# underdoc-wang/ST-MGCN

Hardware: AMD Instinct MI355X
Metric: train_samples_per_sec (higher is better)
Workload: dtype bf16; 1 GPU; model=ST_MGCN, preset=bench-1024, n_nodes=1024, seq_len=8, m_graphs=3, lstm_hidden=64, gcn_hidden=64, global_batch=32, parallelism=dp1, hipgraph=True, impl=hip

## Files before the change

### stmgcn_amd/csrc/wgrad.hip

```cpp

#include "common.h"

namespace {

template <int RB>
__device__ __forceinline__ int tswz(int g, int off) {
  return g * RB + (off ^ ((((unsigned)g / (256 / RB)) & (RB / 16 - 1)) << 4));
}

template <typename T, int RB>
__device__ __forceinline__ typename Frag8<T>::type frag_from(
    const char* lds_tile, int g, int koff_bytes) {
  return *(const typename Frag8<T>::type*)&lds_tile[tswz<RB>(g, koff_bytes)];
}

}

template <typename T>
struct LstmFin {
  unsigned* tickets;
  T* out;
  int gru, cin;
};

__host__ __device__ inline long lstm_grads_layer_off(int l, int GH, int cin) {
  return l == 0 ? 0 : (long)GH * (cin + 64 + 2) + (long)(l - 1) * GH * (64 + 64 + 2);
}

template <typename T, bool FIN>
__global__ void __launch_bounds__(512, 1)
lstm_wgrad_kernel(const T* __restrict__ dA, const T* __restrict__ hseq,
                  const T* __restrict__ x, float* __restrict__ dwih,
                  float* __restrict__ dwhh, float* __restrict__ db,
                  long R, long S_pad, int S, int Tst, int L, int cin1,
                  long tpc, LstmFin<T> fin) {
  using frag = typename Frag8<T>::type;
  constexpr int NTHR = 512;
  constexpr int MTG = 2;
  constexpr int KT = 64;
  constexpr int HT = 64 * 2 * KT;
  extern __shared__ char lds[];

  const int layer = blockIdx.y;
  const int wv = threadIdx.x >> 6, lane = threadIdx.x & 63;
  const int l16 = lane & 15, lgrp = lane >> 4;
  const int gw = wv * 32;
  const long ntile = R / SEQ_TILE;
  const long tb0 = (long)blockIdx.x * tpc;
  const long tb1 = (tb0 + tpc < ntile) ? tb0 + tpc : ntile;
  const long tp0 = S_pad / SEQ_TILE;
  if (!FIN && tb0 >= tb1) return;

  const T* dA_l = dA + (long)layer * R * STM_DA_GATES;
  const T* hp_l = hseq + (long)layer * R * 64;
  const T* hx_l = (layer > 0) ? hseq + (long)(layer - 1) * R * 64 : nullptr;
  const bool l0 = layer == 0;
  const bool x1 = cin1 && l0;

  f32x4 acc_hh[MTG][4], acc_ih[MTG][4];
  float dbp[MTG];
  #pragma unroll
  for (int mt = 0; mt < MTG; ++mt) {
    #pragma unroll
    for (int nt = 0; nt < 4; ++nt) acc_hh[mt][nt] = f32x4{0.f, 0.f, 0.f, 0.f};
    #pragma unroll
    for (int nt = 0; nt < 4; ++nt) acc_ih[mt][nt] = f32x4{0.f, 0.f, 0.f, 0.f};
    dbp[mt] = 0.f;
  }

  const int scb = threadIdx.x & 7, sp = (threadIdx.x >> 3) & 31;
  const int skh = sp >> 4, srow = stm_da_rho(2 * (sp & 15));
  const int sop = threadIdx.x >> 8;

  auto load_h = [&](long tb, frag v[2]) {
    const frag fz = {};
    const long tile = tb + skh;
    const long r = tile * SEQ_TILE + srow;
    v[0] = fz; v[1] = fz;
    if (tile >= tb1) return;
    if (sop == 0) {
      if (tile >= tp0) {
        v[0] = *(const frag*)&hp_l[(r - S_pad) * 64 + scb * 8];
        v[1] = *(const frag*)&hp_l[(r + 1 - S_pad) * 64 + scb * 8];
      }
    } else if (!l0) {
      v[0] = *(const frag*)&hx_l[r * 64 + scb * 8];
      v[1] = *(const frag*)&hx_l[(r + 1) * 64 + scb * 8];
    } else {
      const long s_ = r % S_pad, t_ = r / S_pad;
      if (x1) {
        if (scb == 0) {
          if (s_ < S) ((T*)&v[0])[0] = x[s_ * Tst + t_];
          if (s_ + 1 < S) ((T*)&v[1])[0] = x[(s_ + 1) * Tst + t_];
        }
      } else {
        if (s_ < S) v[0] = *(const frag*)&x[(s_ * Tst + t_) * 64 + scb * 8];
        if (s_ + 1 < S)
          v[1] = *(const frag*)&x[((s_ + 1) * Tst + t_) * 64 + scb * 8];
      }
    }
  };
  auto commit_h = [&](char* buf, const frag v[2]) {
    char* tileT = buf + sop * HT;
    #pragma unroll
    for (int j = 0; j < 8; ++j) {
      union { T t2[2]; int i; } pk;
      pk.t2[0] = ((const T*)&v[0])[j];
      pk.t2[1] = ((const T*)&v[1])[j];
      *(int*)&tileT[tswz<2 * KT>(scb * 8 + j, sp * 4)] = pk.i;
    }
  };
  auto load_a = [&](long tb, frag a[2][MTG]) {
    const frag fz = {};
    #pragma unroll
    for (int kh = 0; kh < 2; ++kh)
      #pragma unroll
      for (int mt = 0; mt < MTG; ++mt) {
        a[kh][mt] = fz;
        if (tb + kh < tb1)
          a[kh][mt] = *(const frag*)&dA_l[stm_da_tile_off((tb + kh) * SEQ_TILE) +
                                          stm_da_elem(gw + mt * 16 + l16, 8 * lgrp)];
      }
  };

  auto kstep = [&](long tb, char* buf, frag vs[2], frag a[2][MTG]) {
    char* hpT = buf;
    char* hxT = buf + HT;
    commit_h(buf, vs);
    load_h(tb + 4, vs);
    __syncthreads();
    #pragma unroll
    for (int kh = 0; kh < 2; ++kh) {
      const int koff = kh * KT + lgrp * 16;
      frag bh[4], bx[4];
      #pragma unroll
      for (int nt = 0; nt < 4; ++nt) bh[nt] = frag_from<T, 2 * KT>(hpT, nt * 16 + l16, koff);
      #pragma unroll
      for (int nt = 0; nt < 4; ++nt) bx[nt] = frag_from<T, 2 * KT>(hxT, nt * 16 + l16, koff);
      #pragma unroll
      for (int mt = 0; mt < MTG; ++mt) {
        const frag af = a[kh][mt];
        #pragma unroll
        for (int nt = 0; nt < 4; ++nt)
          acc_hh[mt][nt] = mfma16x16x32(af, bh[nt], acc_hh[mt][nt]);
        #pragma unroll
        for (int nt = 0; nt < 4; ++nt)
          acc_ih[mt][nt] = mfma16x16x32(af, bx[nt], acc_ih[mt][nt]);
        float sa = 0.f;
        #pragma unroll
        for (int j = 0; j < 8; ++j) sa += (float)af[j];
        dbp[mt] += sa;
      }
    }
    load_a(tb + 4, a);
  };

  frag vs0[2], vs1[2], a0[2][MTG], a1[2][MTG];
  load_h(tb0, vs0);
  load_a(tb0, a0);
  load_h(tb0 + 2, vs1);
  load_a(tb0 + 2, a1);
  for (long tb = tb0; tb < tb1; tb += 4) {
    kstep(tb, lds, vs0, a0);
    if (tb + 2 < tb1) kstep(tb + 2, lds + 2 * HT, vs1, a1);
  }


  float* whh = dwhh + (long)layer * 256 * 64;
  float* wih = dwih + (long)layer * 256 * 64;
  #pragma unroll
  for (int mt = 0; mt < MTG; ++mt) {
    #pragma unroll
    for (int nt = 0; nt < 4; ++nt)
      #pragma unroll
      for (int rr = 0; rr < 4; ++rr) {
        const int m = gw + mt * 16 + lgrp * 4 + rr;
        const int n = nt * 16 + l16;
        unsafeAtomicAdd(&whh[m * 64 + n], acc_hh[mt][nt][rr]);
        if (!x1 || n == 0)
          unsafeAtomicAdd(&wih[m * 64 + n], acc_ih[mt][nt][rr]);
      }
    float v = dbp[mt];
    v += __shfl_xor(v, 16, 64);
    v += __shfl_xor(v, 32, 64);
    if (lgrp == 0) unsafeAtomicAdd(&db[layer * 256 + gw + mt * 16 + l16], v);
  }

  if constexpr (FIN) {
    if (!stm_last_arriver(&fin.tickets[layer], gridDim.x, (int*)lds)) return;
    const int GH = fin.gru ? 192 : 256;
    const int cin_l = l0 ? fin.cin : 64;
    auto row_ih = [&](int m) { return m < GH ? m : -1; };
    auto row_hh = [&](int m) {
      return !fin.gru ? m : (m < 128 ? m : (m >= 192 ? m - 64 : -1));
    };
    T* o_ih = fin.out + lstm_grads_layer_off(layer, GH, fin.cin);
    T* o_hh = o_ih + (long)GH * cin_l;
    T* o_bi = o_hh + (long)GH * 64;
    T* o_bh = o_bi + GH;
    const float* dbl = db + layer * 256;
    constexpr int IT = 256 * 16 / NTHR;
    const bool dense = cin_l == 64;
    const int mb = threadIdx.x;
    float4 vh[IT], vi[IT];
    #pragma unroll
    for (int k = 0; k < IT; ++k) {
      const int i = threadIdx.x + k * NTHR;
      vh[k] = *(const float4*)&whh[i * 4];
      vi[k] = dense ? *(const float4*)&wih[i * 4] : float4{0.f, 0.f, 0.f, 0.f};
    }
    const float vb = mb < 256 ? dbl[mb] : 0.f;
    const float vc = (!dense && mb < 256) ? wih[mb * 64] : 0.f;
    #pragma unroll
    for (int k = 0; k < IT; ++k) {
      const int i = threadIdx.x + k * NTHR;
      const int m = i >> 4, n4 = (i & 15) * 4;
      const int rh = row_hh(m), ri = row_ih(m);
      if (rh >= 0)
        stm_store4<T>(&o_hh[rh * 64 + n4], vh[k].x, vh[k].y, vh[k].z, vh[k].w);
      if (dense && ri >= 0)
        stm_store4<T>(&o_ih[ri * 64 + n4], vi[k].x, vi[k].y, vi[k].z, vi[k].w);
    }
    if (mb >= 256) return;
    const int ri = row_ih(mb), rh = row_hh(mb);
    if (ri >= 0) o_bi[ri] = fromF<T>(vb);
    if (rh >= 0) o_bh[rh] = fromF<T>(vb);
    if (!dense && ri >= 0) o_ih[ri] = fromF<T>(vc);
  }
}

static void lstm_wgrad_launch(void* stream, int dtype, const void* dA,
                              const void* hseq, const void* x, float* dwih,
                              float* dwhh, float* db, long R, long S_pad,
                              int S, int Tst, int L, int cin,
                              unsigned* tickets, void* out, int gru) {
  static long env_chunks = -1;
  if (env_chunks < 0) {
    const char* e = getenv("STMGCN_WGRAD_CHUNKS");
    env_chunks = e ? atol(e) : 0;
  }
  if (R <= 0 || R % SEQ_TILE != 0) {
    printf("stmgcn_lstm_wgrad: R=%ld is not a whole number of dA tiles\n", R);
    return;
  }
  const long ntile = R / SEQ_TILE;
  const long target = env_chunks > 0 ? env_chunks : 512 / (L > 0 ? L : 1);
  long nchunks = (R + 1023) / 1024;
  if (nchunks > target) nchunks = target;
  if (nchunks < 1) nchunks = 1;
  const long tpc = (ntile + nchunks - 1) / nchunks;
  nchunks = (ntile + tpc - 1) / tpc;
  const size_t lds = 2 * 2 * 8192;
  stm_dispatch_lowp("stmgcn_lstm_wgrad", dtype, [&](auto t) {
    using T = decltype(t);
    const LstmFin<T> fin{tickets, (T*)out, gru, cin};
    stm_dispatch_bool(out != nullptr, [&](auto finc) {
      hipLaunchKernelGGL((lstm_wgrad_kernel<T, decltype(finc)::value>),
                         dim3((unsigned)nchunks, L), dim3(512), lds,
                         (hipStream_t)stream, (const T*)dA, (const T*)hseq,
                         (const T*)x, dwih, dwhh, db, R, S_pad, S, Tst, L,
                         cin == 1 ? 1 : 0, tpc, fin);
    });
  });
}

extern "C" void stmgcn_lstm_wgrad(void* stream, int dtype, const void* dA,
                                  const void* hseq, const void* x, float* dwih,
                                  float* dwhh, float* db, long R, long S_pad,
                                  int S, int Tst, int L, int cin) {
  lstm_wgrad_launch(stream, dtype, dA, hseq, x, dwih, dwhh, db, R, S_pad, S,
                    Tst, L, cin, nullptr, nullptr, 0);
}

extern "C" void stmgcn_lstm_wgrad_grads(void* stream, int dtype, const void* dA,
                                        const void* hseq, const void* x,
                                        float* dwih, float* dwhh, float* db,
                                        unsigned* tickets, void* out, long R,
                                        long S_pad, int S, int Tst, int L,
                                        int cin, int gru) {
  lstm_wgrad_launch(stream, dtype, dA, hseq, x, dwih, dwhh, db, R, S_pad, S,
                    Tst, L, cin, tickets, out, gru);
}

struct AtbSrc { const void* a[4]; };

template <typename T>
struct AtbFin {
  unsigned* ticket;
  T *dW, *dbo;
};

template <typename T, bool FIN>
__global__ void __launch_bounds__(256, 1)
atb_wgrad_kernel(AtbSrc As, int CA, const T* __restrict__ B,
                 float* __restrict__ C, float* __restrict__ db,
                 long rows, int M, int N, AtbFin<T> fin) {
  using frag = typename Frag8<T>::type;
  constexpr int KT = 64;
  constexpr int AT_B = 256 * 2 * KT;
  constexpr int BT_B = 64 * 2 * KT;
  constexpr int BUF_B = AT_B + BT_B;
  constexpr int NUA = 4;
  extern __shared__ char lds[];
  float* red = (float*)lds;
  const int wv = threadIdx.x >> 6, lane = threadIdx.x & 63;
  const int l16 = lane & 15, lgrp = lane >> 4;
  const long chunk = (rows + gridDim.x - 1) / gridDim.x;
  const long r0 = (long)blockIdx.x * chunk;
  const long r1 = (r0 + chunk < rows) ? r0 + chunk : rows;
  const int mtiles = (M + 15) / 16;
  const int ntiles = (N + 15) / 16;
  const int mt_mine = (mtiles - wv + 3) / 4;

  f32x4 acc[4][4];
  #pragma unroll
  for (int i = 0; i < 4; ++i)
    #pragma unroll
    for (int nt = 0; nt < 4; ++nt) acc[i][nt] = f32x4{0.f, 0.f, 0.f, 0.f};
  float dbp[8];
  #pragma unroll
  for (int j = 0; j < 8; ++j) dbp[j] = 0.f;

  const int ncba = mtiles * 2, ncbb = ntiles * 2;
  const T* ap[NUA];
  int apair[NUA], acb[NUA];
  #pragma unroll
  for (int i = 0; i < NUA; ++i) {
    const int u = threadIdx.x + i * 256;
    apair[i] = u / ncba; acb[i] = u % ncba;
    ap[i] = nullptr;
    if (u < 32 * ncba && acb[i] * 8 < M)
      ap[i] = (const T*)As.a[(acb[i] * 8) / CA] + (acb[i] * 8) % CA;
  }
  const int bpair = threadIdx.x / ncbb, bcb = threadIdx.x % ncbb;
  const bool bunit = threadIdx.x < 32 * ncbb;
  const T* bp = (bunit && bcb * 8 < N) ? B + bcb * 8 : nullptr;

  struct Regs { frag a[NUA][2]; frag b[2]; };
  auto load_tiles = [&](long kt, Regs& g) {
    const frag fz = {};
    #pragma unroll
    for (int i = 0; i < NUA; ++i) {
      g.a[i][0] = fz; g.a[i][1] = fz;
      const long ra = kt + apair[i] * 2;
      if (ap[i] != nullptr) {
        if (ra < r1) g.a[i][0] = *(const frag*)&ap[i][ra * CA];
        if (ra + 1 < r1) g.a[i][1] = *(const frag*)&ap[i][(ra + 1) * CA];
      }
    }
    g.b[0] = fz; g.b[1] = fz;
    const long rb = kt + bpair * 2;
    if (bp != nullptr) {
      if (rb < r1) g.b[0] = *(const frag*)&bp[rb * N];
      if (rb + 1 < r1) g.b[1] = *(const frag*)&bp[(rb + 1) * N];
    }
  };
  auto commit_tiles = [&](char* buf, const Regs& g) {
    char* AT = buf;
    char* BT = buf + AT_B;
    #pragma unroll
    for (int i = 0; i < NUA; ++i) {
      if (threadIdx.x + i * 256 < 32 * ncba) {
        #pragma unroll
        for (int j = 0; j < 8; ++j) {
          union { T t2[2]; int i; } pk;
          pk.t2[0] = ((const T*)&g.a[i][0])[j];
          pk.t2[1] = ((const T*)&g.a[i][1])[j];
          *(int*)&AT[tswz<2 * KT>(acb[i] * 8 + j, apair[i] * 4)] = pk.i;
        }
      }
    }
    if (bunit) {
      #pragma unroll
      for (int j = 0; j < 8; ++j) {
        union { T t2[2]; int i; } pk;
        pk.t2[0] = ((const T*)&g.b[0])[j];
        pk.t2[1] = ((const T*)&g.b[1])[j];
        *(int*)&BT[tswz<2 * KT>(bcb * 8 + j, bpair * 4)] = pk.i;
        if (db) dbp[j] += toF<T>(pk.t2[0]) + toF<T>(pk.t2[1]);
      }
    }
  };

  auto kstep = [&](long kt, char* buf, Regs& g) {
    commit_tiles(buf, g);
    load_tiles(kt + 2 * KT, g);
    __syncthreads();
    const char* AT = buf;
    const char* BT = buf + AT_B;
    #pragma unroll
    for (int kh = 0; kh < 2; ++kh) {
      const int koff = kh * KT + lgrp * 16;
      frag bf[4];
      #pragma unroll
      for (int nt = 0; nt < 4; ++nt)
        if (nt < ntiles) bf[nt] = frag_from<T, 2 * KT>(BT, nt * 16 + l16, koff);
      #pragma unroll
      for (int i = 0; i < 4; ++i) {
        if (i < mt_mine) {
          const frag a = frag_from<T, 2 * KT>(AT, (wv + i * 4) * 16 + l16, koff);
          #pragma unroll
          for (int nt = 0; nt < 4; ++nt)
            if (nt < ntiles) acc[i][nt] = mfma16x16x32(a, bf[nt], acc[i][nt]);
        }
      }
    }
  };

  Regs g0, g1;
  load_tiles(r0, g0);
  load_tiles(r0 + KT, g1);
  for (long kt = r0; kt < r1; kt += 2 * KT) {
    kstep(kt, lds, g0);
    if (kt + KT < r1) kstep(kt + KT, lds + BUF_B, g1);
  }
  __syncthreads();

  #pragma unroll
  for (int i = 0; i < 4; ++i) {
    if (i >= mt_mine) continue;
    const int mt = wv + i * 4;
    #pragma unroll
    for (int nt = 0; nt < 4; ++nt) {
      if (nt >= ntiles) continue;
      #pragma unroll
      for (int rr = 0; rr < 4; ++rr) {
        const int m = mt * 16 + lgrp * 4 + rr, n = nt * 16 + l16;
        if (m < M && n < N) unsafeAtomicAdd(&C[(long)m * N + n], acc[i][nt][rr]);
      }
    }
  }

  if (db) {
    #pragma unroll
    for (int j = 0; j < 8; ++j) red[threadIdx.x * 8 + j] = bunit ? dbp[j] : 0.f;
    __syncthreads();
    if (threadIdx.x < N) {
      const int n = threadIdx.x, cb = n >> 3, j = n & 7;
      float v = 0.f;
      for (int k = 0; k < 32; ++k) v += red[(k * ncbb + cb) * 8 + j];
      unsafeAtomicAdd(&db[n], v);
    }
  }

  if constexpr (FIN) {
    if (!stm_last_arriver(fin.ticket, gridDim.x, (int*)lds)) return;
    const int n4s = M * N / 4;
    for (int i0 = threadIdx.x; i0 < n4s; i0 += 4 * 256) {
      float4 v[4];
      #pragma unroll
      for (int k = 0; k < 4; ++k) {
        const int i = i0 + k * 256;
        v[k] = i < n4s ? *(const float4*)&C[i * 4] : float4{0.f, 0.f, 0.f, 0.f};
      }
      #pragma unroll
      for (int k = 0; k < 4; ++k) {
        const int i = i0 + k * 256;
        if (i < n4s) stm_store4<T>(&fin.dW[i * 4], v[k].x, v[k].y, v[k].z, v[k].w);
      }
    }
    if (db && threadIdx.x < N) fin.dbo[threadIdx.x] = fromF<T>(db[threadIdx.x]);
  }
}

static void atb_wgrad_launch(void* stream, int dtype, const void** As,
                             int nsrc, int CA, const void* B, float* C,
                             float* db, long rows, int N, unsigned* fin_ticket,
                             void* fin_dW, void* fin_db) {
  long nchunks = (rows + 255) / 256;
  if (nchunks > 512) nchunks = 512;
  if (nchunks < 1) nchunks = 1;
  const dim3 grid((unsigned)nchunks), blk(256);
  const size_t lds = 2 * (256 + 64) * 128;
  const int M = nsrc * CA;
  AtbSrc src{};
  for (int i = 0; i < nsrc && i < 4; ++i) src.a[i] = As[i];
  stm_dispatch_lowp("stmgcn_atb_wgrad", dtype, [&](auto t) {
    using T = decltype(t);
    const AtbFin<T> fin{fin_ticket, (T*)fin_dW, (T*)fin_db};
    stm_dispatch_bool(fin_ticket != nullptr, [&](auto finc) {
      STM_CHECK_HIP(hipFuncSetAttribute(
          (const void*)atb_wgrad_kernel<T, decltype(finc)::value>,
          hipFuncAttributeMaxDynamicSharedMemorySize, (int)lds));
      hipLaunchKernelGGL((atb_wgrad_kernel<T, decltype(finc)::value>), grid, blk,
                         lds, (hipStream_t)stream, src, CA, (const T*)B, C, db,
                         rows, M, N, fin);
    });
  });
}

extern "C" void stmgcn_atb_wgrad_multi(void* stream, int dtype, const void** As,
                                       int nsrc, int CA, const void* B, float* C,
                                       float* db, long rows, int N) {
  atb_wgrad_launch(stream, dtype, As, nsrc, CA, B, C, db, rows, N, nullptr,
                   nullptr, nullptr);
}

extern "C" void stmgcn_atb_wgrad_multi_grads(void* stream, int dtype,
                                             const void** As, int nsrc, int CA,
                                             const void* B, float* C, float* db,
                                             unsigned* ticket, void* dW,
                                             void* dbo, long rows, int N) {
  atb_wgrad_launch(stream, dtype, As, nsrc, CA, B, C, db, rows, N, ticket, dW,
                   dbo);
}

extern "C" void stmgcn_atb_wgrad(void* stream_v, int dtype, const void* A,
                                 const void* B, float* C, float* db, long rows,
                                 int M, int N) {
  stmgcn_atb_wgrad_multi(stream_v, dtype, &A, 1, M, B, C, db, rows, N);
}
```

Baseline: 16990 samples/s.

## Specialize LSTM wgrad loads per layer form and interleave LDS reads with MFMA

Splits the LSTM weight-gradient kernel into compile-time forms (scalar layer-0 input, dense layer-0 input, hidden handoff) so the h/x staging loads are branchless, with predicated addresses and masking applied at commit time. Adds sched_barrier fences so LDS fragment reads for the next k-half overlap with MFMAs on the current one. It also halves the default chunk target and drops the env override. The aim is to cut divergent branching and load-latency stalls in the inner loop, at the cost of extra registers and fewer blocks for atomics-based reduction parallelism.

```diff
diff --git a/stmgcn_amd/csrc/wgrad.hip b/stmgcn_amd/csrc/wgrad.hip
--- a/stmgcn_amd/csrc/wgrad.hip
+++ b/stmgcn_amd/csrc/wgrad.hip
@@ -12,6 +12,14 @@
 __device__ __forceinline__ typename Frag8<T>::type frag_from(
     const char* lds_tile, int g, int koff_bytes) {
   return *(const typename Frag8<T>::type*)&lds_tile[tswz<RB>(g, koff_bytes)];
+}
+
+enum : int { WG_SCALAR0 = 0, WG_DENSE0 = 1, WG_HANDOFF = 2 };
+template <typename F>
+__device__ __forceinline__ void wgrad_uniform_form(int form, F&& f) {
+  if (form == WG_SCALAR0) f(std::integral_constant<int, WG_SCALAR0>{});
+  else if (form == WG_DENSE0) f(std::integral_constant<int, WG_DENSE0>{});
+  else f(std::integral_constant<int, WG_HANDOFF>{});
 }
 
 }
@@ -70,101 +78,138 @@
 
   const int scb = threadIdx.x & 7, sp = (threadIdx.x >> 3) & 31;
   const int skh = sp >> 4, srow = stm_da_rho(2 * (sp & 15));
-  const int sop = threadIdx.x >> 8;
-
-  auto load_h = [&](long tb, frag v[2]) {
+  const bool sop = threadIdx.x >= 256;
+
+  struct KSet {
+    frag h[2];
+    unsigned short xs[2];
+    frag a[2][MTG];
+    int live;
+  };
+
+  auto load_h = [&](auto form, long tb, KSet& g) {
+    constexpr int F = decltype(form)::value;
+    const long tile = tb + skh;
+    const bool tin = tile < tb1;
+    const long r = tile * SEQ_TILE + srow;
+    const bool hlive = tin && tile >= tp0 && !(F == WG_SCALAR0 && sop);
+    const T* ph = hlive ? hp_l + (r - S_pad) * 64 : hp_l;
+    const T *p0 = ph, *p1 = ph + 64;
+    bool lv0 = hlive, lv1 = hlive;
+    if constexpr (F == WG_HANDOFF) {
+      const T* px = tin ? hx_l + r * 64 : hx_l;
+      p0 = sop ? px : p0; p1 = sop ? px + 64 : p1;
+      lv0 = lv1 = sop ? tin : hlive;
+    } else {
+      const long t_ = (unsigned)tile / (unsigned)tp0;
+      const long s_ = r - t_ * S_pad;
+      const bool x0 = sop && tin && s_ < S, x1 = sop && tin && s_ + 1 < S;
+      const long e0 = x0 ? s_ * Tst + t_ : 0, e1 = x1 ? (s_ + 1) * Tst + t_ : 0;
+      if constexpr (F == WG_DENSE0) {
+        p0 = sop ? x + e0 * 64 : p0; p1 = sop ? x + e1 * 64 : p1;
+      } else {
+        g.xs[0] = *(const unsigned short*)&x[e0];
+        g.xs[1] = *(const unsigned short*)&x[e1];
+      }
+      lv0 = sop ? x0 : hlive; lv1 = sop ? x1 : hlive;
+    }
+    g.h[0] = *(const frag*)&p0[scb * 8];
+    g.h[1] = *(const frag*)&p1[scb * 8];
+    g.live = (lv0 ? 1 : 0) | (lv1 ? 2 : 0);
+  };
+  auto commit_h = [&](auto form, char* buf, const KSet& g) {
+    constexpr int F = decltype(form)::value;
     const frag fz = {};
-    const long tile = tb + skh;
-    const long r = tile * SEQ_TILE + srow;
-    v[0] = fz; v[1] = fz;
-    if (tile >= tb1) return;
-    if (sop == 0) {
-      if (tile >= tp0) {
-        v[0] = *(const frag*)&hp_l[(r - S_pad) * 64 + scb * 8];
-        v[1] = *(const frag*)&hp_l[(r + 1 - S_pad) * 64 + scb * 8];
-      }
-    } else if (!l0) {
-      v[0] = *(const frag*)&hx_l[r * 64 + scb * 8];
-      v[1] = *(const frag*)&hx_l[(r + 1) * 64 + scb * 8];
-    } else {
-      const long s_ = r % S_pad, t_ = r / S_pad;
-      if (x1) {
-        if (scb == 0) {
-          if (s_ < S) ((T*)&v[0])[0] = x[s_ * Tst + t_];
-          if (s_ + 1 < S) ((T*)&v[1])[0] = x[(s_ + 1) * Tst + t_];
-        }
-      } else {
-        if (s_ < S) v[0] = *(const frag*)&x[(s_ * Tst + t_) * 64 + scb * 8];
-        if (s_ + 1 < S)
-          v[1] = *(const frag*)&x[((s_ + 1) * Tst + t_) * 64 + scb * 8];
-      }
-    }
-  };
-  auto commit_h = [&](char* buf, const frag v[2]) {
-    char* tileT = buf + sop * HT;
+    char* tileT = buf + (sop ? HT : 0);
+    const frag v0 = (g.live & 1) ? g.h[0] : fz;
+    const frag v1 = (g.live & 2) ? g.h[1] : fz;
+    const int xw = ((g.live & 1) ? (int)g.xs[0] : 0) |
+                   ((g.live & 2) ? (int)g.xs[1] << 16 : 0);
     #pragma unroll
     for (int j = 0; j < 8; ++j) {
-      union { T t2[2]; int i; } pk;
-      pk.t2[0] = ((const T*)&v[0])[j];
-      pk.t2[1] = ((const T*)&v[1])[j];
-      *(int*)&tileT[tswz<2 * KT>(scb * 8 + j, sp * 4)] = pk.i;
-    }
-  };
-  auto load_a = [&](long tb, frag a[2][MTG]) {
-    const frag fz = {};
+      union { typename Frag8<T>::elem t2[2]; int i; } pk;
+      pk.t2[0] = v0[j];
+      pk.t2[1] = v1[j];
+      int w = pk.i;
+      if constexpr (F == WG_SCALAR0) w = sop ? ((j == 0 && scb == 0) ? xw : 0) : w;
+      *(int*)&tileT[tswz<2 * KT>(scb * 8 + j, sp * 4)] = w;
+    }
+  };
+  auto load_a = [&](long tb, KSet& g) {
     #pragma unroll
     for (int kh = 0; kh < 2; ++kh)
       #pragma unroll
       for (int mt = 0; mt < MTG; ++mt) {
-        a[kh][mt] = fz;
-        if (tb + kh < tb1)
-          a[kh][mt] = *(const frag*)&dA_l[stm_da_tile_off((tb + kh) * SEQ_TILE) +
-                                          stm_da_elem(gw + mt * 16 + l16, 8 * lgrp)];
-      }
-  };
-
-  auto kstep = [&](long tb, char* buf, frag vs[2], frag a[2][MTG]) {
+        const long off = stm_da_tile_off((tb + kh) * SEQ_TILE) +
+                         stm_da_elem(gw + mt * 16 + l16, 8 * lgrp);
+        g.a[kh][mt] = *(const frag*)&dA_l[tb + kh < tb1 ? off : 0];
+      }
+  };
+
+  auto kstep = [&](auto form, long tb, char* buf, KSet& g) {
     char* hpT = buf;
     char* hxT = buf + HT;
-    commit_h(buf, vs);
-    load_h(tb + 4, vs);
+    commit_h(form, buf, g);
+    __builtin_amdgcn_sched_barrier(0);
+    load_h(form, tb + 4, g);
+    __builtin_amdgcn_sched_barrier(0);
     __syncthreads();
-    #pragma unroll
-    for (int kh = 0; kh < 2; ++kh) {
-      const int koff = kh * KT + lgrp * 16;
-      frag bh[4], bx[4];
-      #pragma unroll
-      for (int nt = 0; nt < 4; ++nt) bh[nt] = frag_from<T, 2 * KT>(hpT, nt * 16 + l16, koff);
-      #pragma unroll
-      for (int nt = 0; nt < 4; ++nt) bx[nt] = frag_from<T, 2 * KT>(hxT, nt * 16 + l16, koff);
-      #pragma unroll
-      for (int mt = 0; mt < MTG; ++mt) {
-        const frag af = a[kh][mt];
+    const frag fz = {};
+    frag bh[2][4], bx[2][4], af[2][MTG];
+    auto read_b = [&](frag (&b)[4], const char* tileT, int kh) {
+      #pragma unroll
+      for (int nt = 0; nt < 4; ++nt)
+        b[nt] = frag_from<T, 2 * KT>(tileT, nt * 16 + l16, kh * KT + lgrp * 16);
+    };
+    auto mfma_b = [&](f32x4 (&acc)[MTG][4], const frag (&b)[4], int kh) {
+      #pragma unroll
+      for (int mt = 0; mt < MTG; ++mt)
         #pragma unroll
         for (int nt = 0; nt < 4; ++nt)
-          acc_hh[mt][nt] = mfma16x16x32(af, bh[nt], acc_hh[mt][nt]);
-        #pragma unroll
-        for (int nt = 0; nt < 4; ++nt)
-          acc_ih[mt][nt] = mfma16x16x32(af, bx[nt], acc_ih[mt][nt]);
+          acc[mt][nt] = mfma16x16x32(af[kh][mt], b[nt], acc[mt][nt]);
+    };
+    #pragma unroll
+    for (int kh = 0; kh < 2; ++kh)
+      #pragma unroll
+      for (int mt = 0; mt < MTG; ++mt)
+        af[kh][mt] = tb + kh < tb1 ? g.a[kh][mt] : fz;
+    read_b(bh[0], hpT, 0);
+    read_b(bx[0], hxT, 0);
+    __builtin_amdgcn_sched_barrier(0);
+    mfma_b(acc_hh, bh[0], 0);
+    read_b(bh[1], hpT, 1);
+    __builtin_amdgcn_sched_barrier(0);
+    mfma_b(acc_ih, bx[0], 0);
+    read_b(bx[1], hxT, 1);
+    __builtin_amdgcn_sched_barrier(0);
+    mfma_b(acc_hh, bh[1], 1);
+    mfma_b(acc_ih, bx[1], 1);
+    #pragma unroll
+    for (int kh = 0; kh < 2; ++kh)
+      #pragma unroll
+      for (int mt = 0; mt < MTG; ++mt) {
         float sa = 0.f;
         #pragma unroll
-        for (int j = 0; j < 8; ++j) sa += (float)af[j];
+        for (int j = 0; j < 8; ++j) sa += (float)af[kh][mt][j];
         dbp[mt] += sa;
       }
-    }
-    load_a(tb + 4, a);
-  };
-
-  frag vs0[2], vs1[2], a0[2][MTG], a1[2][MTG];
-  load_h(tb0, vs0);
-  load_a(tb0, a0);
-  load_h(tb0 + 2, vs1);
-  load_a(tb0 + 2, a1);
-  for (long tb = tb0; tb < tb1; tb += 4) {
-    kstep(tb, lds, vs0, a0);
-    if (tb + 2 < tb1) kstep(tb + 2, lds + 2 * HT, vs1, a1);
-  }
-
+    __builtin_amdgcn_sched_barrier(0);
+    load_a(tb + 4, g);
+  };
+
+  wgrad_uniform_form(l0 ? (cin1 ? WG_SCALAR0 : WG_DENSE0) : WG_HANDOFF, [&](auto form) {
+    KSet g0, g1;
+    load_h(form, tb0, g0);
+    load_a(tb0, g0);
+    load_h(form, tb0 + 2, g1);
+    load_a(tb0 + 2, g1);
+    long tb = tb0;
+    do {
+      kstep(form, tb, lds, g0);
+      kstep(form, tb + 2, lds + 2 * HT, g1);
+      tb += 4;
+    } while (tb < tb1);
+  });
 
   float* whh = dwhh + (long)layer * 256 * 64;
   float* wih = dwih + (long)layer * 256 * 64;
@@ -234,17 +279,16 @@
                               float* dwhh, float* db, long R, long S_pad,
                               int S, int Tst, int L, int cin,
                               unsigned* tickets, void* out, int gru) {
-  static long env_chunks = -1;
-  if (env_chunks < 0) {
-    const char* e = getenv("STMGCN_WGRAD_CHUNKS");
-    env_chunks = e ? atol(e) : 0;
-  }
   if (R <= 0 || R % SEQ_TILE != 0) {
     printf("stmgcn_lstm_wgrad: R=%ld is not a whole number of dA tiles\n", R);
     return;
   }
   const long ntile = R / SEQ_TILE;
-  const long target = env_chunks > 0 ? env_chunks : 512 / (L > 0 ? L : 1);
+  if (ntile >= (1L << 31)) {
+    printf("stmgcn_lstm_wgrad: R=%ld has too many dA tiles\n", R);
+    return;
+  }
+  const long target = 256 / (L > 0 ? L : 1);
   long nchunks = (R + 1023) / 1024;
   if (nchunks > target) nchunks = target;
   if (nchunks < 1) nchunks = 1;
```

New measurement: 17520 samples/s, median of 6. 1.03x the previous value.
